# CESNET/GPUJPEG

Measured on AMD Instinct MI355X. Metric: Mpix/s encode+decode (8K RGB q75), higher is better.
Workload: dtype f32

## Files before the change

### gpujpeg_amd/csrc/gj_dec_entropy_tok.hip

```cpp
#include "gj_dec_internal.h"
#include "gj_bitreader.h"

#ifndef GJ_TOK_SUB
#define GJ_TOK_SUB 16
#define GJ_TOK_SUB_MAX 20
#endif
#define GJ_TOK_MAX_SUBS (GJ_TOK_CAP_U / GJ_TOK_SUB + (GJ_TOK_SUB <= 17 ? GJ_TOK_GMAX / 2 : GJ_TOK_GMAX))
#define GJ_TOK_WSTAGE 944
#define GJ_TOK_WG_PER_CU 4
#ifndef GJ_TOK_SYNC
#define GJ_TOK_SYNC 48
#endif
#define GJ_TOK_CHUNK_MAX 48

#ifdef GJ_TRACE_PHASES
static __device__ unsigned long long* gj_trace_buf;
extern "C" GJ_HIP_API int gj_hip_trace_set(void* p) { return hipMemcpyToSymbol(HIP_SYMBOL(gj_trace_buf), &p, sizeof p) == hipSuccess ? 0 : -1; }
#define GJ_TRACE(slot) do { if (threadIdx.x == 0 && gj_trace_buf) gj_trace_buf[(size_t)blockIdx.x * 16 + (slot)] = __builtin_amdgcn_s_memrealtime(); } while (0)
#else
#define GJ_TRACE(slot) ((void)0)
#endif

#ifdef GJ_TOK_STATS
extern "C" GJ_HIP_API unsigned long long gj_tok_stats[64];
unsigned long long gj_tok_stats[64];
#define GJ_STAT_WAVE(sm, i, lane, sym) do { gj_wave_sync(); (sm).statsym[threadIdx.x] = (sym); gj_wave_sync(); if ((lane) == 0) { \
    unsigned long long s_ = 0, m_ = 0; for (int q_ = 0; q_ < 64; q_++) { const unsigned v_ = (sm).statsym[(threadIdx.x & ~63) + q_]; s_ += v_; if (v_ > m_) m_ = v_; } \
    GJ_STAT(i, s_); GJ_STAT((i) + 1, 64 * m_); GJ_STAT((i) + 2, 1); } } while (0)
#define GJ_SYMS(c) (((c) >> 16) + 2u * ((c) & 0xFFFFu))
#define GJ_STAT(i, n) __atomic_fetch_add(&gj_tok_stats[i], (unsigned long long)(n), __ATOMIC_RELAXED)
#else
#define GJ_STAT(i, n) ((void)0)
#define GJ_STAT_WAVE(sm, i, lane, sym) ((void)0)
#endif

#ifndef GJ_TOK_WIN
#define GJ_TOK_WIN 1
#endif
#if GJ_TOK_WIN == 1
#define GJ_TOK_WIN_INIT(sm, p1) uint32_t wcur_ = (p1) >> 5, w0_ = (sm).U[wcur_], w1_ = (sm).U[wcur_ + 1], wnx_ = 0
#define GJ_TOK_WIN_BITS(sm, p1) wnx_ = (sm).U[wcur_ + 2]; const uint32_t win = __builtin_amdgcn_alignbit(w0_, w1_, ~(p1))
#define GJ_TOK_WIN_STEP(p1) do { const uint32_t wn_ = (p1) >> 5; const bool cross_ = wn_ != wcur_; w0_ = cross_ ? w1_ : w0_; w1_ = cross_ ? wnx_ : w1_; wcur_ = wn_; } while (0)
#else
#define GJ_TOK_WIN_INIT(sm, p1) ((void)0)
#define GJ_TOK_WIN_BITS(sm, p1) const uint32_t wi = (p1) >> 5; const uint32_t win = __builtin_amdgcn_alignbit((sm).U[wi], (sm).U[wi + 1], ~(p1))
#define GJ_TOK_WIN_STEP(p1) ((void)0)
#endif


struct GjTokLds {
    uint32_t U[GJ_TOK_CAP_U / 4 + 8];
    __attribute__((aligned(16))) uint16_t tab[2 * GJ_DEC2_WORDS];
    __attribute__((aligned(8))) uint2 rec[GJ_TOK_MAX_SUBS];
    __attribute__((aligned(16))) uint16_t pool[(GJ_TOK_MAX_BLOCKS + GJ_TOK_GMAX) * 2 + 4 * GJ_TOK_WSTAGE];
    uint32_t bb[GJ_TOK_GMAX + 1], cap[GJ_TOK_GMAX + 1], first[GJ_TOK_GMAX];
    uint16_t tabsel[GJ_TOK_GMAX];
    uint32_t sbit[GJ_TOK_GMAX], ebit[GJ_TOK_GMAX], sub0[GJ_TOK_GMAX + 1];
    uint32_t tmp[4];
    uint32_t nwork[2], big;
    uint32_t gpos;
    uint8_t zz[64 + 64];
#ifdef GJ_TOK_STATS
    uint32_t statsym[256];
#endif
};

__device__ __forceinline__ uint32_t gj_tok_run_in(const GjTokLds& sm, const uint32_t from, const uint32_t start_bit)
{
    uint32_t p1 = from - 1u;
    const uint32_t e1 = start_bit - 1u;
    uint32_t z = 1;
    uint32_t toff = (uint32_t)GJ_DEC2_WORDS * 2u;
    GJ_TOK_WIN_INIT(sm, p1);
    while (p1 < e1) {
        GJ_TOK_WIN_BITS(sm, p1);
        const uint16_t* t = reinterpret_cast<const uint16_t*>(reinterpret_cast<const uint8_t*>(sm.tab) + toff);
        uint32_t e = t[gj_bfe_u32<32 - GJ_DEC_FAST_BITS, GJ_DEC_FAST_BITS>(win)];
        if ((e & 31u) == 0) e = t[(e >> 5) + ((win >> 16) & 63u)];
        p1 += e & 31u;
        GJ_TOK_WIN_STEP(p1);
        z += (e >> 9) & 63u;
        const uint32_t inside = (uint32_t)((int32_t)(z - 64u) >> 31);
        z &= inside;
        toff = ((uint32_t)GJ_DEC2_WORDS * 2u) & inside;
    }
    return (p1 - e1) | (z << 5);
}

template <int MODE>
__device__ __forceinline__ uint32_t gj_tok_decode(const GjTokLds& sm, const uint32_t start_bit, const uint32_t end_bit, const uint32_t entry, uint32_t& counts,
                                                  uint16_t* __restrict__ tok_out ,
                                                  uint32_t* __restrict__ s_blkinfo ,
                                                  const uint32_t tok_rel , uint32_t blk,
                                                  const uint32_t nblocks, int16_t* __restrict__ coefs ,
                                                  uint32_t* __restrict__ s_big)
{
    uint32_t p1 = start_bit + (entry & 31u) - 1u;
    const uint32_t e1 = end_bit - 1u;
    uint32_t z = (entry >> 5) & 63u;
    uint32_t toff = z == 0 ? 0u : (uint32_t)GJ_DEC2_WORDS * 2u;
    uint32_t nb = 0, ntok = 0, mx = 0;
    uint16_t* tp = tok_out;
    GJ_TOK_WIN_INIT(sm, p1);
    while (p1 < e1) {
        GJ_TOK_WIN_BITS(sm, p1);
        const uint16_t* t = reinterpret_cast<const uint16_t*>(reinterpret_cast<const uint8_t*>(sm.tab) + toff);
        uint32_t e = t[gj_bfe_u32<32 - GJ_DEC_FAST_BITS, GJ_DEC_FAST_BITS>(win)];
        if ((e & 31u) == 0) e = t[(e >> 5) + ((win >> 16) & 63u)];
        const uint32_t tot = e & 31u, adv = (e >> 9) & 63u, sz = (e >> 5) & 15u;
        if (MODE == 0) {
            ntok += e >> 15;
        } else {
            const uint32_t x = win << (tot - sz);
            uint32_t neg = (uint32_t)((int32_t)~x >> 31);
            GJ_KEEP(neg);
            const uint32_t mag = (x ^ neg) >> ((32u - sz) & 31u);
            const int v = (int)((mag ^ neg) - neg);
            if ((int16_t)e < 0) {
                const uint32_t pos = z + adv - 1u;
                if (MODE == 1) {
                    mx = max(mx, sz);
                    *tp++ = (uint16_t)(((uint32_t)v << 6) | sm.zz[pos]);
                } else {
                    if (blk + nb < nblocks && pos < 64u) coefs[(uint64_t)(blk + nb) * 64 + sm.zz[pos]] = (int16_t)v;
                    ntok++;
                }
            } else if (z == 0) {
                const uint32_t t = MODE == 1 ? tok_rel + (uint32_t)(tp - tok_out) : tok_rel + ntok;
                if (blk + nb <= nblocks) s_blkinfo[blk + nb] = (sz ? (uint32_t)v & 0xFFFFu : 0u) | (t << 16);
            }
        }
        p1 += tot;
        GJ_TOK_WIN_STEP(p1);
        z += adv;
        const uint32_t inside = (uint32_t)((int32_t)(z - 64u) >> 31);
        z &= inside;
        toff = ((uint32_t)GJ_DEC2_WORDS * 2u) & inside;
        nb += 1u + inside;
    }
    if (MODE == 1) ntok = (uint32_t)(tp - tok_out);
    if (MODE == 1 && mx >= 10u) *s_big = 1u;
    counts = nb | (ntok << 16);
    return (p1 - e1) | (z << 5);
}

template <bool COOP>
__global__ __launch_bounds__(256, GJ_TOK_WG_PER_CU) void k_huffman_decode_tok(const gj_geom g, const uint8_t* __restrict__ jpeg, uint64_t jpeg_size,
                                                               const uint32_t* __restrict__ seg_pos, const uint32_t* __restrict__ seg_len,
                                                               const uint32_t* __restrict__ seg_index, const int seg_count_max,
                                                               const uint32_t* __restrict__ seg_count_ptr, const GjBatchPlan plan,
                                                               const uint16_t* __restrict__ tabs, int16_t* __restrict__ coefs,
                                                               uint16_t* __restrict__ d_tok, const uint32_t tok_cap, uint2* __restrict__ d_rec,
                                                               uint32_t* __restrict__ overflow, const GjFold F)
{
    constexpr int CAP_U = GJ_TOK_CAP_U, MAX_BLOCKS = GJ_TOK_MAX_BLOCKS, GMAX = GJ_TOK_GMAX, MAX_SUBS = GJ_TOK_MAX_SUBS;
    if (g.fb.sizes != nullptr) {
        const size_t z = blockIdx.z;
        jpeg += z * g.fb.jpeg;
        jpeg_size = g.fb.sizes[z];
        seg_pos += z * g.fb.seg; seg_len += z * g.fb.seg; seg_index += z * g.fb.seg;
        if (seg_count_ptr) seg_count_ptr += z * (sizeof(gj_scan_summary) / 4);
        overflow += z * (sizeof(gj_scan_summary) / 4);
        coefs += z * g.fb.coefs; d_tok += z * g.fb.tok; d_rec += z * g.fb.rec;
    }
    __shared__ GjTokLds sm;
    constexpr int POOL = sizeof(sm.pool) / 2;
    uint32_t* const s_stage = sm.U + 1;
    uint16_t* const s_pool = sm.pool;
    uint32_t* const s_blkinfo = reinterpret_cast<uint32_t*>(sm.pool);
    uint2* const s_rec = sm.rec;
    uint32_t *const s_bb = sm.bb, *const s_cap = sm.cap, *const s_first = sm.first, *const s_sbit = sm.sbit, *const s_ebit = sm.ebit, *const s_sub0 = sm.sub0;
    uint32_t* const s_tmp = sm.tmp;
    constexpr int BORROW = ((4 * GMAX + 1) * 2 + 7) & ~7;
    uint32_t* const s_pos = reinterpret_cast<uint32_t*>(s_pool + POOL - BORROW);
    uint32_t* const s_len = s_pos + GMAX;
    uint32_t* const s_ubyte = s_len + GMAX;
    uint32_t* const s_ulen = s_ubyte + GMAX + 1;
    static_assert(BORROW <= GJ_TOK_WSTAGE && MAX_SUBS <= POOL - BORROW, "borrowed space");
    uint16_t* const s_work = s_pool;

    const int tid = threadIdx.x, lane = tid & 63, wave = tid >> 6;
    GJ_TRACE(0);
    uint32_t sel_of_lane = 0x0C0C0C0Cu;
    {
        int at = 3;
#pragma unroll
        for (int k = 0; k < 4; k++)
            if (lane & (1 << k)) { sel_of_lane = (sel_of_lane & ~(0xFFu << (8 * at))) | ((uint32_t)k << (8 * at)); at--; }
    }
    if (tid < 128) sm.zz[tid] = tid < 64 ? GJ_ZZ[tid] : 0;
    if (tid == 0) sm.U[0] = 0;
    const uint32_t* end = reinterpret_cast<const uint32_t*>((reinterpret_cast<uintptr_t>(jpeg) + jpeg_size + 3) & ~(uintptr_t)3);

    int pc = 0;
    while (pc + 1 < plan.n && (int)blockIdx.x >= plan.batch0[pc + 1]) pc++;
    const int G = plan.g[pc];
    const int si0 = plan.first[pc] + ((int)blockIdx.x - plan.batch0[pc]) * G;
    uint32_t ld_s = 0xFFFFFFFFu, ld_p = 0, ld_l = 0;
    if (F.recs == nullptr && tid < G && si0 + tid < seg_count_max) { ld_s = seg_index[si0 + tid]; ld_p = seg_pos[si0 + tid]; ld_l = seg_len[si0 + tid]; }
    const int seg_count = seg_count_ptr ? min((int)*seg_count_ptr, seg_count_max) : seg_count_max;
    if (si0 >= seg_count) return;
    const int nseg = min(min(G, plan.first[pc] + plan.count[pc] - si0), seg_count - si0);
    if (F.recs != nullptr) {
        static_assert(GJ_FOLD_SCRATCH_WORDS(GJ_TOK_GMAX) * 2 <= (GJ_TOK_MAX_BLOCKS + GJ_TOK_GMAX) * 2, "fold scratch inside the block slots");
        if (!gj_fold_batch<GJ_TOK_GMAX>(F, g, jpeg, jpeg_size, plan, pc, si0, nseg, reinterpret_cast<uint32_t*>(sm.pool), s_tmp, ld_s, ld_p, ld_l)) return;
    }
    uint32_t loaded_tabs = 0xFFFFFFFFu;
    auto load_tables = [&](const uint32_t tb) {
        const uint4* src0 = reinterpret_cast<const uint4*>(tabs + (tb & 0xFFu) * GJ_DEC2_WORDS);
        const uint4* src1 = reinterpret_cast<const uint4*>(tabs + (tb >> 8) * GJ_DEC2_WORDS);
        uint4* dst = reinterpret_cast<uint4*>(sm.tab);
        for (int t = tid; t < GJ_DEC2_WORDS / 8; t += 256) { dst[t] = src0[t]; dst[GJ_DEC2_WORDS / 8 + t] = src1[t]; }
        loaded_tabs = tb;
    };
    if (plan.n > 1 && plan.n == g.comp_count) load_tables((uint32_t)(g.comp[pc].dc_table * 2 + 0) | ((uint32_t)(g.comp[pc].ac_table * 2 + 1) << 8));
    uint32_t my_pos = 0, my_len = 0, my_nblk = 0;
    {
        uint32_t first = 0, tb = 0;
        if (tid < nseg) {
            const uint32_t s = ld_s, p_ = ld_p, l_ = ld_l;
            if (s < (uint32_t)g.segment_count) {
                const GjSeg sg = gj_segment(g, (int)s);
                const gj_comp_geom& kc = g.comp[sg.comp];
                my_nblk = (uint32_t)sg.nblocks;
                my_pos = p_;
                my_len = l_;
                first = (uint32_t)(kc.data_offset / 64) + (uint32_t)sg.mcu_first;
                tb = (uint32_t)(kc.dc_table * 2 + 0) | ((uint32_t)(kc.ac_table * 2 + 1) << 8);
                if (((my_len + 3u) & ~3u) + 8u > (uint32_t)CAP_U || my_nblk > (uint32_t)MAX_BLOCKS) {
                    *overflow = 1u;
                    my_len = 0;
                    my_nblk = 0;
                }
            }
        }
        if (tid < GMAX) {
            s_first[tid] = first;
            sm.tabsel[tid] = (uint16_t)tb;
        }
        if (wave == 0) {
            s_bb[tid + 1] = gj_wave_incl_scan(tid < nseg ? my_nblk + 1u : 0u);
            s_cap[tid + 1] = gj_wave_incl_scan(my_len ? ((my_len + 3u) & ~3u) + 8u : 0u);
        }
        if (tid == 0) { s_bb[0] = 0; s_cap[0] = 0; sm.nwork[0] = 0; sm.nwork[1] = 0; }
    }
    static_assert(GMAX == 64, "one wave holds the batch's segment table");
    __syncthreads();
    const uint32_t stage0 = (2u * s_bb[nseg] + 7u) & ~7u, stage_cap = (((uint32_t)POOL - stage0) >> 2) & ~7u;
    uint16_t* const stage = s_pool + stage0 + (uint32_t)wave * stage_cap;

    for (int j0 = 0; j0 < nseg;) {
        if (tid == 0) sm.big = 0;
        if (tid < nseg) { s_pos[tid] = my_pos; s_len[tid] = my_len; }
        {
            const unsigned long long mb = __ballot(lane >= j0 && lane < nseg && my_nblk != 0u);
            if (wave == 0 && lane == (mb ? (int)__builtin_ctzll(mb) : j0)) sm.gpos = my_pos;
        }
        const uint32_t tb = sm.tabsel[j0];
        const bool other = lane > j0 && lane < nseg && s_bb[lane + 1] - s_bb[lane] != 1u && sm.tabsel[lane] != tb;
        const unsigned long long mo = __ballot(other);
        const int jstop = mo ? (int)__builtin_ctzll(mo) : nseg;
        const unsigned long long mf = __ballot(lane + 1 > j0 && lane + 1 <= jstop && s_cap[lane + 1] - s_cap[j0] <= (uint32_t)CAP_U);
        const int j1 = max(j0 + 1, mf ? 64 - (int)__builtin_clzll(mf) : 0);
        const int ng = j1 - j0;
        if (COOP) {
            const uint32_t n16 = min((s_cap[j1] - s_cap[j0] + 16u + 4u + 15u) >> 4, (uint32_t)(sizeof(sm.U) / 16));
            uint4* const z = reinterpret_cast<uint4*>(sm.U);
            for (uint32_t t = (uint32_t)tid; t < n16; t += 256u) z[t] = uint4{0u, 0u, 0u, 0u};
        }
        __syncthreads();
        GJ_TRACE(1);

        if (tb != loaded_tabs) load_tables(tb);

        bool coop = false;
        if (COOP) {
            bool irregular = false;
            if (lane < ng) {
                const int j = j0 + lane;
                irregular = s_len[j] == 0 || (lane + 1 < ng && s_pos[j + 1] != s_pos[j] + s_len[j] + 2u);
            }
            const uint32_t A = s_pos[j0], total = s_pos[j1 - 1] + s_len[j1 - 1] - A;
            coop = __ballot(irregular) == 0ull && total <= 256u * GJ_TOK_CHUNK_MAX && A >= 8u && (uint64_t)A + total <= jpeg_size;
        }
        if (coop) {
            const uint32_t A = s_pos[j0], total = s_pos[j1 - 1] + s_len[j1 - 1] - A;
            const uint32_t C = (((total + 255u) >> 8) + 3u) & ~3u;
            const uint32_t off0 = (uint32_t)tid * C;
            const uintptr_t a = reinterpret_cast<uintptr_t>(jpeg) + A + off0;
            const uint32_t* src = reinterpret_cast<const uint32_t*>(a & ~(uintptr_t)3) - 1;
            const uint32_t lead = (uint32_t)((reinterpret_cast<uintptr_t>(jpeg) + A) & 3);
            uint32_t win[GJ_TOK_CHUNK_MAX / 4 + 3];
#pragma unroll
            for (int i = 0; i < GJ_TOK_CHUNK_MAX / 4 + 3; i++) {
                win[i] = 0;
                if ((uint32_t)i < C / 4 + 3u && off0 < total + 4u && src + i < end) win[i] = src[i];
            }
            constexpr int ND = GJ_TOK_CHUNK_MAX / 4;
            uint64_t keep = 0, mark = 0;
            {
                const uint32_t K7 = 0x7F7F7F7Fu, K8 = 0x80808080u;
                uint32_t eq_prev = 0, m2_prev = 0, st_prev = 0;
                uint32_t ffc = 0;
                if (off0 != 0) {
                    const uint32_t x = __builtin_amdgcn_alignbyte(win[1], win[0], lead);
                    ffc = ((x & K7) + 0x01010101u) & x & K8;
                }
#pragma unroll
                for (int i = 0; i <= ND; i++) {
                    if ((uint32_t)(4 * i) <= C) {
                        const uint32_t x = __builtin_amdgcn_alignbyte(win[i + 2], win[i + 1], lead);
                        const uint32_t t = x & K7;
                        const uint32_t eq = (t + 0x01010101u) & x & K8;
                        const uint32_t zr = ~((t + K7) | x) & K8;
                        const uint32_t y = (x ^ 0xD0D0D0D0u) & 0xF8F8F8F8u;
                        const uint32_t rz = ~(((y & K7) + K7) | y) & K8;
                        const uint32_t before = __builtin_amdgcn_alignbit(eq, ffc, 24);
                        ffc = eq;
                        const uint32_t m2 = before & rz, st = before & zr;
                        if (i > 0) {
                            const uint32_t m1 = eq_prev & __builtin_amdgcn_alignbit(m2, m2_prev, 8);
                            const uint32_t kp = K8 & ~(st_prev | m2_prev | m1);
                            keep |= (uint64_t)((((kp >> 7) * 0x01020408u) >> 24) & 15u) << (4 * (i - 1));
                            mark |= (uint64_t)((((m1 >> 7) * 0x01020408u) >> 24) & 15u) << (4 * (i - 1));
                        }
                        eq_prev = eq; m2_prev = m2; st_prev = st;
                    }
                }
                const uint32_t nvalid = off0 >= total ? 0u : min(total - off0, C);
                const uint64_t valid = nvalid >= 64u ? ~0ull : (1ull << nvalid) - 1ull;
                keep &= valid;
                mark &= valid;
            }
            const uint32_t nkeep = (uint32_t)__popcll(keep), nmark = (uint32_t)__popcll(mark);
            uint32_t tot;
            const uint32_t inc = gj_wg256_incl_scan(nkeep | (nmark << 16), s_tmp, &tot);
            uint32_t o = (inc & 0xFFFFu) - nkeep, m = (inc >> 16) - nmark;
            coop = (tot >> 16) == (uint32_t)(ng - 1);
            if (coop) {
#pragma unroll
                for (int i = 0; i < ND; i++) {
                    if ((uint32_t)(4 * i) < C) {
                        const uint32_t x = __builtin_amdgcn_alignbyte(win[i + 2], win[i + 1], lead);
                        const uint32_t nk = (uint32_t)(keep >> (4 * i)) & 15u, nm = (uint32_t)(mark >> (4 * i)) & 15u;
                        const uint32_t below = nm ? ((nm & (0u - nm)) - 1u) : 15u;
                        const uint32_t nA = nk & below, nB = nk & ~below;
                        const uint32_t cA = (uint32_t)__popc(nA);
                        const uint32_t compA = __builtin_amdgcn_perm(0u, x, (uint32_t)__builtin_amdgcn_ds_bpermute((int)(nA << 2), (int)sel_of_lane));
                        const uint32_t compB = __builtin_amdgcn_perm(0u, x, (uint32_t)__builtin_amdgcn_ds_bpermute((int)(nB << 2), (int)sel_of_lane));
                        const uint32_t pA = o + 8u * m, pB = pA + cA + 8u;
                        const uint32_t shA = 8u * (pA & 3u), shB = 8u * (pB & 3u);
                        uint32_t* const dA = s_stage + (pA >> 2);
                        uint32_t* const dB = s_stage + (pB >> 2);
                        atomicOr(dA, compA >> shA);
                        atomicOr(dA + 1, __builtin_amdgcn_alignbit(compA, 0u, shA));
                        atomicOr(dB, compB >> shB);
                        atomicOr(dB + 1, __builtin_amdgcn_alignbit(compB, 0u, shB));
                        uint32_t mm = m;
                        for (uint32_t q = nm; q; q &= q - 1u) {
                            mm++;
                            s_ubyte[j0 + (int)mm] = o + (uint32_t)__popc(nk & ((q & (0u - q)) - 1u)) + 8u * mm;
                        }
                        m = mm;
                        o += (uint32_t)__popc(nk);
                    }
                }
                if (tid == 255) s_ubyte[j1] = o + 8u * m + 8u;
                if (tid == 0) s_ubyte[j0] = 0;
            }
        }
        __syncthreads();
        if (tid == 0) GJ_STAT(coop ? 30 : 31, 1);
        if (coop) {
            if (tid >= j0 && tid < j1) s_ulen[tid] = s_ubyte[tid + 1] - s_ubyte[tid] - 8u;
        } else {
            for (int j = j0 + wave; j < j1; j += 4) {
                const uint32_t len = s_len[j], base = s_cap[j] - s_cap[j0];
                uint32_t ulen = 0;
                if (len) {
                    const uintptr_t a = reinterpret_cast<uintptr_t>(jpeg) + s_pos[j];
                    const uint32_t* src = reinterpret_cast<const uint32_t*>(a & ~(uintptr_t)3);
                    const uint32_t ndw = ((uint32_t)(a & 3) + len + 3u) >> 2;
                    uint32_t w0 = 0;
                    if ((uint32_t)lane < ndw && src + lane < end) w0 = src[lane];
                    ulen = gj_unstuff_segment(jpeg, end, s_pos[j], len, s_stage, base, lane, w0);
                }
                if (lane == 0) { s_ubyte[j] = base; s_ulen[j] = ulen; }
            }
        }
        __syncthreads();

        GJ_TRACE(2);
        uint32_t sub_bytes = GJ_TOK_SUB;
        {
            uint32_t ulen = 0;
            if (tid >= j0 && tid < j1) {
                ulen = my_nblk ? s_ulen[tid] : 0u;
                s_sbit[tid] = s_ubyte[tid] * 8u + 32u;
                s_ebit[tid] = (s_ubyte[tid] + ulen) * 8u + 32u;
            }
            uint32_t tot;
            uint32_t a = gj_wg256_incl_scan(((ulen + GJ_TOK_SUB - 1) / GJ_TOK_SUB) | (ulen << 16), s_tmp, &tot) & 0xFFFFu;
            const uint32_t passes = ((tot & 0xFFFFu) + 255u) >> 8, bytes = tot >> 16;
            if (passes >= 2) {
#pragma unroll
                for (uint32_t s = GJ_TOK_SUB + 1; s <= GJ_TOK_SUB_MAX; s++)
                    if (sub_bytes == GJ_TOK_SUB && bytes / s + (uint32_t)ng <= 256u * (passes - 1u)) sub_bytes = s;
            }
            sub_bytes = (uint32_t)__builtin_amdgcn_readfirstlane((int)sub_bytes);
            if (sub_bytes != GJ_TOK_SUB) a = gj_wg256_incl_scan((ulen + sub_bytes - 1u) / sub_bytes, s_tmp, &tot);
            if (tid >= j0 && tid < j1) s_sub0[tid + 1] = min(a, (uint32_t)MAX_SUBS);
            if (tid == 0) s_sub0[j0] = 0;
        }
        __syncthreads();
        const int nsub = (int)s_sub0[j1];
        const uint32_t sub_bits = sub_bytes * 8u;
        if (tid == 0) { GJ_STAT(32 + min(nsub / 32, 31), 1); GJ_STAT(28, sub_bytes != GJ_TOK_SUB ? 1 : 0); }
        for (int k = tid; k < nsub; k += 256) {
            int lo = j0, hi = j1;
            while (hi - lo > 1) {
                const int mid = (lo + hi) >> 1;
                if (s_sub0[mid] <= (uint32_t)k) lo = mid; else hi = mid;
            }
            s_rec[k].x = (uint32_t)lo << 22;
        }
        __syncthreads();

        GJ_TRACE(3);
        for (int k0 = 0; k0 < nsub; k0 += 256) {
            const int k = k0 + tid;
            uint32_t c0 = 0;
            if (k < nsub) {
                const int j = (int)(s_rec[k].x >> 22);
                const uint32_t i = (uint32_t)k - s_sub0[j];
                const uint32_t sb = s_sbit[j] + i * sub_bits, eb = min(sb + sub_bits, s_ebit[j]);
                const uint32_t e0 = i == 0 ? 0u : gj_tok_run_in(sm, sb - (uint32_t)GJ_TOK_SYNC, sb);
                const uint32_t x0 = gj_tok_decode<0>(sm, sb, eb, e0, c0, nullptr, nullptr, 0, 0, 0, nullptr, nullptr);
                s_rec[k] = make_uint2(e0 | (x0 << 11) | ((uint32_t)j << 22), c0);
            }
            GJ_STAT_WAVE(sm, 16, lane, GJ_SYMS(c0));
        }
        GJ_TRACE(4);
        for (int round = 0;; round++) {
            __syncthreads();
            uint32_t* const cnt = &sm.nwork[round & 1];
            for (int k0 = 0; k0 < nsub; k0 += 256) {
                const int k = k0 + tid;
                bool cand = false;
                if (k < nsub) {
                    const uint32_t x = s_rec[k].x;
                    cand = (uint32_t)k != s_sub0[x >> 22] && ((s_rec[k - 1].x >> 11) & 0x7FFu) != (x & 0x7FFu);
                }
                const unsigned long long m = __ballot(cand);
                uint32_t base = 0;
                if (lane == 0 && m) base = atomicAdd(cnt, (uint32_t)__popcll(m));
                base = (uint32_t)__builtin_amdgcn_readfirstlane((int)base);
                if (cand) s_work[base + (uint32_t)__popcll(m & ((1ull << lane) - 1ull))] = (uint16_t)k;
            }
            __syncthreads();
            const int nwork = (int)*cnt;
            if (tid == 0) { GJ_STAT(0, round == 0 ? nsub : 0); GJ_STAT(1 + min(round, 13), nwork); GJ_STAT(15, nwork == 0 ? round : 0); }
            if (tid == 0) sm.nwork[(round + 1) & 1] = 0;
            if (nwork == 0) break;
            for (int w = tid; w < nwork; w += 256) {
                const int k = s_work[w];
                const int j = (int)(s_rec[k].x >> 22);
                const uint32_t i = (uint32_t)k - s_sub0[j];
                const uint32_t sb = s_sbit[j] + i * sub_bits, eb = min(sb + sub_bits, s_ebit[j]);
                const uint32_t e = (s_rec[k - 1].x >> 11) & 0x7FFu;
                uint32_t c;
                const uint32_t x = gj_tok_decode<0>(sm, sb, eb, e, c, nullptr, nullptr, 0, 0, 0, nullptr, nullptr);
                s_rec[k] = make_uint2(e | (x << 11) | ((uint32_t)j << 22), c);
            }
        }

        GJ_TRACE(5);
        {
            uint32_t carry = 0;
            for (int k0 = 0; k0 < nsub; k0 += 256) {
                const int k = k0 + tid;
                const uint32_t v = k < nsub ? s_rec[k].y : 0;
                uint32_t tot;
                const uint32_t inc = gj_wg256_incl_scan(v, s_tmp, &tot);
                __syncthreads();
                if (k < nsub) s_rec[k].y = carry + inc;
                carry += tot;
            }
        }
        for (uint32_t b = s_bb[j0] + (uint32_t)tid; b < s_bb[j1]; b += 256) s_blkinfo[b] = 0xFFFF0000u;
        __syncthreads();

        GJ_TRACE(6);
        const uint32_t T = nsub > 0 ? s_rec[nsub - 1].y >> 16 : 0u;
        uint32_t gbase = 4u * sm.gpos;
        if (sm.gpos > tok_cap / 4u || T > tok_cap - gbase) gbase = 0xFFFFFFFFu;
        if (gbase != 0xFFFFFFFFu) {
            const int ka = (int)(((uint32_t)nsub * (uint32_t)wave) >> 2), kb = (int)(((uint32_t)nsub * (uint32_t)(wave + 1)) >> 2);
            for (int k0 = ka; k0 < kb;) {
                const uint32_t P0 = k0 > 0 ? s_rec[k0 - 1].y >> 16 : 0u;
                const uint32_t a0 = (gbase + P0) & 7u;
                const int kk = k0 + lane;
                const bool fits = kk < kb && a0 + ((s_rec[min(kk, nsub - 1)].y >> 16) - P0) <= stage_cap;
                const unsigned long long fm = __ballot(fits);
                const int n = fm == ~0ull ? 64 : __builtin_ctzll(~fm);
                gj_wave_sync();
                uint32_t c = 0;
                if (lane < n) {
                    const int j = (int)(s_rec[kk].x >> 22);
                    const uint32_t kf = s_sub0[j];
                    const uint32_t i = (uint32_t)kk - kf;
                    const uint32_t before_k = kk > 0 ? s_rec[kk - 1].y : 0u, before_f = kf > 0 ? s_rec[kf - 1].y : 0u;
                    const uint32_t sb = s_sbit[j] + i * sub_bits, eb = min(sb + sub_bits, s_ebit[j]);
                    gj_tok_decode<1>(sm, sb, eb, s_rec[kk].x & 0x7FFu, c, stage + a0 + ((before_k >> 16) - P0), s_blkinfo + s_bb[j], before_k >> 16,
                                     (before_k & 0xFFFFu) - (before_f & 0xFFFFu), s_bb[j + 1] - s_bb[j] - 1u, nullptr, &sm.big);
                }
                gj_wave_sync();
                GJ_STAT_WAVE(sm, 20, lane, GJ_SYMS(c));
                const uint32_t cnt = (s_rec[k0 + n - 1].y >> 16) - P0;
                uint16_t* const dst = d_tok + (size_t)(gbase + P0 - a0);
                for (uint32_t p = (uint32_t)lane; p * 8u < a0 + cnt; p += 64) {
                    const uint32_t lo = p * 8u, hi = lo + 8u;
                    if (lo >= a0 && hi <= a0 + cnt) {
                        *reinterpret_cast<uint4*>(dst + lo) = *reinterpret_cast<const uint4*>(stage + lo);
                    } else {
                        for (uint32_t s = max(lo, a0); s < min(hi, a0 + cnt); s++) dst[s] = stage[s];
                    }
                }
                k0 += n;
                if (lane == 0) { GJ_STAT(24, 1); GJ_STAT(25, n); GJ_STAT(26, k0 >= kb ? (kb - ka + 63) / 64 : 0); GJ_STAT(27, k0 >= kb ? 1 : 0); }
            }
        }
        __syncthreads();

        GJ_TRACE(7);
        const bool planes = sm.big != 0 || gbase == 0xFFFFFFFFu;
        if (planes) {
            for (int j = j0 + wave; j < j1; j += 4) {
                const uint32_t chunks = (s_bb[j + 1] - s_bb[j] - 1u) * 8u;
                for (uint32_t c = (uint32_t)lane; c < chunks; c += 64)
                    reinterpret_cast<uint4*>(coefs + (uint64_t)(s_first[j] + (c >> 3)) * 64)[c & 7u] = make_uint4(0, 0, 0, 0);
            }
            __syncthreads();
            for (int k = tid; k < nsub; k += 256) {
                const int j = (int)(s_rec[k].x >> 22);
                const uint32_t kf = s_sub0[j];
                const uint32_t i = (uint32_t)k - kf;
                const uint32_t before_k = k > 0 ? s_rec[k - 1].y : 0u, before_f = kf > 0 ? s_rec[kf - 1].y : 0u;
                const uint32_t sb = s_sbit[j] + i * sub_bits, eb = min(sb + sub_bits, s_ebit[j]);
                uint32_t c;
                gj_tok_decode<2>(sm, sb, eb, s_rec[k].x & 0x7FFu, c, nullptr, s_blkinfo + s_bb[j], 0, (before_k & 0xFFFFu) - (before_f & 0xFFFFu),
                                 s_bb[j + 1] - s_bb[j] - 1u, coefs + (uint64_t)s_first[j] * 64, nullptr);
            }
            __syncthreads();
        }

        for (int j = j0 + wave; j < j1; j += 4) {
            const uint32_t bb = s_bb[j];
            const int nblk = (int)(s_bb[j + 1] - bb) - 1;
            const uint32_t k_end = s_sub0[j + 1];
            const uint32_t seg_end = k_end > s_sub0[j] ? s_rec[k_end - 1].y >> 16 : 0u;
            int carry = 0;
            for (int kb0 = 0; kb0 < nblk; kb0 += 64) {
                const int kb = kb0 + lane;
                const uint32_t info = kb < nblk ? s_blkinfo[bb + kb] : 0xFFFF0000u;
                const uint32_t inc = gj_wave_incl_scan((uint32_t)(int)(int16_t)(info & 0xFFFFu));
                const int dc = carry + (int)inc;
                carry += (int)(uint32_t)__builtin_amdgcn_readlane((int)inc, 63);
                if (kb < nblk) {
                    const uint32_t r = s_first[j] + (uint32_t)kb;
                    if (planes) {
                        coefs[(uint64_t)r * 64] = (int16_t)dc;
                        d_rec[r] = make_uint2(0u, 0xFFFF0000u);
                    } else {
                        const uint32_t t0 = info >> 16, nx = s_blkinfo[bb + kb + 1] >> 16;
                        const uint32_t t1 = nx != 0xFFFFu ? nx : seg_end;
                        const bool seen = t0 != 0xFFFFu;
                        const uint32_t cnt = seen && t1 >= t0 ? min(t1 - t0, 63u) : 0u;
                        d_rec[r] = make_uint2(seen ? gbase + t0 : 0u, (cnt << 16) | ((uint32_t)dc & 0xFFFFu));
                    }
                }
            }
        }
        __syncthreads();
        GJ_TRACE(8);
        j0 = j1;
    }
}

void gj_launch_huffman_tok(const gj_dec_job* job, hipStream_t st)
{
    const gj_geom& g = job->g;
    const unsigned frames = job->batch.count > 1 ? job->batch.count : 1u;
    const GjBatchPlan plan = gj_plan_batches(job, GJ_TOK_CAP_U, GJ_TOK_MAX_BLOCKS, GJ_TOK_GMAX, frames > 1 ? 0u : GJ_TOK_RESIDENT);
    auto kernel = job->tune.dec_tok_nocoop ? k_huffman_decode_tok<false> : k_huffman_decode_tok<true>;
    GjFold F = {nullptr, nullptr, 0, 0, 0, nullptr, nullptr};
    const bool fold = gj_tok_folds_table(job);
    if (fold) {
        const gj_scan_deferred& sc = job->scan;
        F = GjFold{sc.recs, sc.lists, sc.wgs, sc.part_bytes, sc.begin, sc.h_summary, sc.h_maxlen_parts};
        *sc.maxlen_part_count = (uint32_t)plan.batch0[plan.n];
    }
    hipLaunchKernelGGL(kernel, dim3((unsigned)plan.batch0[plan.n], 1, frames), dim3(256), 0, st, g, job->d_jpeg, job->jpeg_size, job->d_seg_pos, job->d_seg_len, job->d_seg_index,
                       job->seg_count, fold ? nullptr : job->d_seg_count, plan, job->d_huff_tab2, job->d_coefs, (uint16_t*)job->d_tok, job->tok_cap, (uint2*)job->d_blkrec,
                       job->d_overflow, F);
}

bool gj_tok_folds_table(const gj_dec_job* job)
{
    const gj_geom& g = job->g;
    if (!job->scan.valid || job->batch.count > 1 || g.fb.sizes != nullptr || g.interleaved || g.restart_interval <= 0 || job->seg_count != g.segment_count) return false;
    if (job->scan.wgs > 256u || job->scan.h_summary == nullptr || job->scan.h_maxlen_parts == nullptr || job->scan.maxlen_part_count == nullptr) return false;
    const GjBatchPlan plan = gj_plan_batches(job, GJ_TOK_CAP_U, GJ_TOK_MAX_BLOCKS, GJ_TOK_GMAX, GJ_TOK_RESIDENT);
    return plan.n == g.comp_count && (uint32_t)plan.batch0[plan.n] <= job->scan.maxlen_capacity;
}
```

Measured before the change: 171,400.

## Interleave two sub-stream Huffman counting passes per thread in token decoder

When a group holds more than 256 sub-streams, the first counting pass now gives each thread two sub-streams and decodes them in lockstep within one loop. This replaces several serial 256-wide rounds, cutting the trip count and giving the LDS table lookups two independent chains to overlap. In exchange it adds register pressure, extra work for a frozen reader once its stream ends, and divergence when the two streams differ in length. Step-count tracing and extra stats hooks are also added, but they compile out by default.

```diff
diff --git a/gpujpeg_amd/csrc/gj_dec_entropy_tok.hip b/gpujpeg_amd/csrc/gj_dec_entropy_tok.hip
--- a/gpujpeg_amd/csrc/gj_dec_entropy_tok.hip
+++ b/gpujpeg_amd/csrc/gj_dec_entropy_tok.hip
@@ -12,26 +12,52 @@
 #define GJ_TOK_SYNC 48
 #endif
 #define GJ_TOK_CHUNK_MAX 48
+#ifndef GJ_TOK_PAIR
+#define GJ_TOK_PAIR 1
+#endif
+#ifndef GJ_TOK_PAIR_MIN
+#define GJ_TOK_PAIR_MIN 256
+#endif
 
 #ifdef GJ_TRACE_PHASES
 static __device__ unsigned long long* gj_trace_buf;
 extern "C" GJ_HIP_API int gj_hip_trace_set(void* p) { return hipMemcpyToSymbol(HIP_SYMBOL(gj_trace_buf), &p, sizeof p) == hipSuccess ? 0 : -1; }
 #define GJ_TRACE(slot) do { if (threadIdx.x == 0 && gj_trace_buf) gj_trace_buf[(size_t)blockIdx.x * 16 + (slot)] = __builtin_amdgcn_s_memrealtime(); } while (0)
+#define GJ_TRACE_STEPS(slot, n) do { const uint32_t m_ = gj_wave_max(n); if (threadIdx.x == 0 && gj_trace_buf) gj_trace_buf[(size_t)blockIdx.x * 16 + (slot)] += m_; } while (0)
+__device__ __forceinline__ uint32_t gj_wave_max(const uint32_t v)
+{
+    uint32_t m = 0;
+    bool in = true;
+    for (int b = 15; b >= 0; b--) {
+        const bool has = in && ((v >> b) & 1u);
+        if (__ballot(has)) { m |= 1u << b; in = has; }
+    }
+    return m;
+}
 #else
 #define GJ_TRACE(slot) ((void)0)
-#endif
-
+#define GJ_TRACE_STEPS(slot, n) ((void)(n))
+#endif
+
+#define GJ_SYMS(c) (((c) >> 16) + 2u * ((c) & 0xFFFFu))
 #ifdef GJ_TOK_STATS
 extern "C" GJ_HIP_API unsigned long long gj_tok_stats[64];
 unsigned long long gj_tok_stats[64];
 #define GJ_STAT_WAVE(sm, i, lane, sym) do { gj_wave_sync(); (sm).statsym[threadIdx.x] = (sym); gj_wave_sync(); if ((lane) == 0) { \
     unsigned long long s_ = 0, m_ = 0; for (int q_ = 0; q_ < 64; q_++) { const unsigned v_ = (sm).statsym[(threadIdx.x & ~63) + q_]; s_ += v_; if (v_ > m_) m_ = v_; } \
     GJ_STAT(i, s_); GJ_STAT((i) + 1, 64 * m_); GJ_STAT((i) + 2, 1); } } while (0)
-#define GJ_SYMS(c) (((c) >> 16) + 2u * ((c) & 0xFFFFu))
 #define GJ_STAT(i, n) __atomic_fetch_add(&gj_tok_stats[i], (unsigned long long)(n), __ATOMIC_RELAXED)
+extern "C" GJ_HIP_API unsigned int gj_tok_nsub_hist[GJ_TOK_MAX_SUBS + 1], gj_tok_pair_passes, gj_tok_plane_groups;
+unsigned int gj_tok_nsub_hist[GJ_TOK_MAX_SUBS + 1], gj_tok_pair_passes, gj_tok_plane_groups;
+#define GJ_STAT_NSUB(n) __atomic_fetch_add(&gj_tok_nsub_hist[n], 1u, __ATOMIC_RELAXED)
+#define GJ_STAT_PAIR() __atomic_fetch_add(&gj_tok_pair_passes, 1u, __ATOMIC_RELAXED)
+#define GJ_STAT_PLANES() __atomic_fetch_add(&gj_tok_plane_groups, 1u, __ATOMIC_RELAXED)
 #else
 #define GJ_STAT(i, n) ((void)0)
-#define GJ_STAT_WAVE(sm, i, lane, sym) ((void)0)
+#define GJ_STAT_NSUB(n) ((void)0)
+#define GJ_STAT_PAIR() ((void)0)
+#define GJ_STAT_PLANES() ((void)0)
+#define GJ_STAT_WAVE(sm, i, lane, sym) ((void)(sym))
 #endif
 
 #ifndef GJ_TOK_WIN
@@ -65,7 +91,7 @@
 #endif
 };
 
-__device__ __forceinline__ uint32_t gj_tok_run_in(const GjTokLds& sm, const uint32_t from, const uint32_t start_bit)
+__device__ __forceinline__ uint32_t gj_tok_run_in(const GjTokLds& sm, const uint32_t from, const uint32_t start_bit, uint32_t& steps )
 {
     uint32_t p1 = from - 1u;
     const uint32_t e1 = start_bit - 1u;
@@ -83,6 +109,7 @@
         const uint32_t inside = (uint32_t)((int32_t)(z - 64u) >> 31);
         z &= inside;
         toff = ((uint32_t)GJ_DEC2_WORDS * 2u) & inside;
+        steps++;
     }
     return (p1 - e1) | (z << 5);
 }
@@ -93,7 +120,7 @@
                                                   uint32_t* __restrict__ s_blkinfo ,
                                                   const uint32_t tok_rel , uint32_t blk,
                                                   const uint32_t nblocks, int16_t* __restrict__ coefs ,
-                                                  uint32_t* __restrict__ s_big)
+                                                  uint32_t* __restrict__ s_big, uint32_t& steps )
 {
     uint32_t p1 = start_bit + (entry & 31u) - 1u;
     const uint32_t e1 = end_bit - 1u;
@@ -137,12 +164,93 @@
         z &= inside;
         toff = ((uint32_t)GJ_DEC2_WORDS * 2u) & inside;
         nb += 1u + inside;
+        steps++;
     }
     if (MODE == 1) ntok = (uint32_t)(tp - tok_out);
     if (MODE == 1 && mx >= 10u) *s_big = 1u;
     counts = nb | (ntok << 16);
     return (p1 - e1) | (z << 5);
 }
+
+#if GJ_TOK_PAIR && GJ_TOK_WIN == 1
+struct GjTokStream {
+    uint32_t from, start, end;
+    uint32_t entry, exit, counts;
+};
+struct GjTokReader { uint32_t p1, z, toff, cnt, w0, w1, wnx, wcur; };
+
+__device__ __forceinline__ void gj_tok_reader_step(GjTokReader& r, const uint32_t e)
+{
+    r.p1 += e & 31u;
+    const uint32_t wn = r.p1 >> 5;
+    const bool cross = wn != r.wcur;
+    r.w0 = cross ? r.w1 : r.w0;
+    r.w1 = cross ? r.wnx : r.w1;
+    r.wcur = wn;
+    r.z += (e >> 9) & 63u;
+    const uint32_t inside = (uint32_t)((int32_t)(r.z - 64u) >> 31);
+    r.z &= inside;
+    r.toff = ((uint32_t)GJ_DEC2_WORDS * 2u) & inside;
+    r.cnt += ((e & 0x8000u) << 1) + 1u + inside;
+}
+
+__device__ __forceinline__ void gj_tok_pair_loop(const GjTokLds& sm, GjTokReader& A, GjTokReader& B, const uint32_t endA1, const uint32_t endB1, uint32_t& steps)
+{
+    static_assert((32 + 8 * GJ_TOK_CAP_U + 30) / 32 + 2 < (int)(sizeof(GjTokLds::U) / 4), "a frozen reader's look-ahead stays in the stage");
+    const uint8_t* const tab = reinterpret_cast<const uint8_t*>(sm.tab);
+    while (A.p1 < endA1 || B.p1 < endB1) {
+        const uint32_t actA = (uint32_t)((int32_t)(A.p1 - endA1) >> 31), actB = (uint32_t)((int32_t)(B.p1 - endB1) >> 31);
+        A.wnx = sm.U[A.wcur + 2];
+        B.wnx = sm.U[B.wcur + 2];
+        const uint32_t winA = __builtin_amdgcn_alignbit(A.w0, A.w1, ~A.p1), winB = __builtin_amdgcn_alignbit(B.w0, B.w1, ~B.p1);
+        const uint16_t* const tA = reinterpret_cast<const uint16_t*>(tab + A.toff);
+        const uint16_t* const tB = reinterpret_cast<const uint16_t*>(tab + B.toff);
+        uint32_t eA = tA[gj_bfe_u32<32 - GJ_DEC_FAST_BITS, GJ_DEC_FAST_BITS>(winA)];
+        uint32_t eB = tB[gj_bfe_u32<32 - GJ_DEC_FAST_BITS, GJ_DEC_FAST_BITS>(winB)];
+        if ((((eA & 31u) == 0) | ((eB & 31u) == 0)) != 0) {
+            if ((eA & 31u) == 0) eA = tA[(eA >> 5) + ((winA >> 16) & 63u)];
+            if ((eB & 31u) == 0) eB = tB[(eB >> 5) + ((winB >> 16) & 63u)];
+        }
+        gj_tok_reader_step(A, eA & actA);
+        gj_tok_reader_step(B, eB & actB);
+        steps++;
+    }
+}
+
+__device__ __forceinline__ void gj_tok_reader_init(const GjTokLds& sm, GjTokReader& r, const GjTokStream& s)
+{
+    r.p1 = s.from - 1u;
+    r.z = s.from != s.start ? 1u : 0u;
+    r.toff = r.z ? (uint32_t)GJ_DEC2_WORDS * 2u : 0u;
+    r.cnt = 0;
+    r.wcur = r.p1 >> 5;
+    r.w0 = sm.U[r.wcur];
+    r.w1 = sm.U[r.wcur + 1];
+    r.wnx = 0;
+}
+
+__device__ __forceinline__ void gj_tok_count2(const GjTokLds& sm, GjTokStream& A, GjTokStream& B, uint32_t& steps)
+{
+    GjTokReader a, b;
+    gj_tok_reader_init(sm, a, A);
+    gj_tok_reader_init(sm, b, B);
+    gj_tok_pair_loop(sm, a, b, A.start - 1u, B.start - 1u, steps);
+    A.entry = (a.p1 - (A.start - 1u)) | (a.z << 5);
+    B.entry = (b.p1 - (B.start - 1u)) | (b.z << 5);
+    a.toff = a.z == 0 ? 0u : (uint32_t)GJ_DEC2_WORDS * 2u;
+    b.toff = b.z == 0 ? 0u : (uint32_t)GJ_DEC2_WORDS * 2u;
+    a.cnt = 0;
+    b.cnt = 0;
+    gj_tok_pair_loop(sm, a, b, A.end - 1u, B.end - 1u, steps);
+    A.exit = (a.p1 - (A.end - 1u)) | (a.z << 5);
+    B.exit = (b.p1 - (B.end - 1u)) | (b.z << 5);
+    A.counts = a.cnt;
+    B.counts = b.cnt;
+}
+#define GJ_TOK_PAIRED 1
+#else
+#define GJ_TOK_PAIRED 0
+#endif
 
 template <bool COOP>
 __global__ __launch_bounds__(256, GJ_TOK_WG_PER_CU) void k_huffman_decode_tok(const gj_geom g, const uint8_t* __restrict__ jpeg, uint64_t jpeg_size,
@@ -415,7 +523,7 @@
         __syncthreads();
         const int nsub = (int)s_sub0[j1];
         const uint32_t sub_bits = sub_bytes * 8u;
-        if (tid == 0) { GJ_STAT(32 + min(nsub / 32, 31), 1); GJ_STAT(28, sub_bytes != GJ_TOK_SUB ? 1 : 0); }
+        if (tid == 0) { GJ_STAT(32 + min(nsub / 32, 31), 1); GJ_STAT(28, sub_bytes != GJ_TOK_SUB ? 1 : 0); GJ_STAT_NSUB(nsub); }
         for (int k = tid; k < nsub; k += 256) {
             int lo = j0, hi = j1;
             while (hi - lo > 1) {
@@ -427,19 +535,60 @@
         __syncthreads();
 
         GJ_TRACE(3);
-        for (int k0 = 0; k0 < nsub; k0 += 256) {
-            const int k = k0 + tid;
-            uint32_t c0 = 0;
-            if (k < nsub) {
-                const int j = (int)(s_rec[k].x >> 22);
-                const uint32_t i = (uint32_t)k - s_sub0[j];
-                const uint32_t sb = s_sbit[j] + i * sub_bits, eb = min(sb + sub_bits, s_ebit[j]);
-                const uint32_t e0 = i == 0 ? 0u : gj_tok_run_in(sm, sb - (uint32_t)GJ_TOK_SYNC, sb);
-                const uint32_t x0 = gj_tok_decode<0>(sm, sb, eb, e0, c0, nullptr, nullptr, 0, 0, 0, nullptr, nullptr);
-                s_rec[k] = make_uint2(e0 | (x0 << 11) | ((uint32_t)j << 22), c0);
-            }
-            GJ_STAT_WAVE(sm, 16, lane, GJ_SYMS(c0));
-        }
+        uint32_t steps1 = 0;
+        for (int b0 = 0; b0 < nsub;) {
+            const int rem = nsub - b0;
+            const int P = rem > 256 ? 256 : (GJ_TOK_PAIRED && rem > GJ_TOK_PAIR_MIN ? (rem + 1) >> 1 : rem);
+            const int n = GJ_TOK_PAIRED ? min(rem, 2 * P) : P;
+            uint32_t syms = 0;
+#if GJ_TOK_PAIRED
+            if (n > P) {
+                if (tid == 0) GJ_STAT_PAIR();
+                if (tid < P) {
+                    const int kA = b0 + tid, kB = kA + P;
+                    const bool hasB = kB < b0 + n;
+                    const int jA = (int)(s_rec[kA].x >> 22);
+                    const uint32_t iA = (uint32_t)kA - s_sub0[jA];
+                    GjTokStream A, B;
+                    A.start = s_sbit[jA] + iA * sub_bits;
+                    A.end = min(A.start + sub_bits, s_ebit[jA]);
+                    A.from = iA == 0 ? A.start : A.start - (uint32_t)GJ_TOK_SYNC;
+                    int jB = 0;
+                    B.from = B.start = B.end = 32u;
+                    if (hasB) {
+                        jB = (int)(s_rec[kB].x >> 22);
+                        const uint32_t iB = (uint32_t)kB - s_sub0[jB];
+                        B.start = s_sbit[jB] + iB * sub_bits;
+                        B.end = min(B.start + sub_bits, s_ebit[jB]);
+                        B.from = iB == 0 ? B.start : B.start - (uint32_t)GJ_TOK_SYNC;
+                    }
+                    gj_tok_count2(sm, A, B, steps1);
+                    s_rec[kA] = make_uint2(A.entry | (A.exit << 11) | ((uint32_t)jA << 22), A.counts);
+                    if (hasB) s_rec[kB] = make_uint2(B.entry | (B.exit << 11) | ((uint32_t)jB << 22), B.counts);
+                    syms = GJ_SYMS(A.counts) + GJ_SYMS(B.counts);
+                    GJ_STAT(19, (iA != 0 && A.end - A.start <= 32u ? 1 : 0) + (hasB && B.from != B.start && B.end - B.start <= 32u ? 1 : 0));
+                    GJ_STAT(23, (iA == 0 && A.end - A.start < (uint32_t)GJ_TOK_SYNC ? 1 : 0) + (hasB && B.from == B.start && B.end - B.start < (uint32_t)GJ_TOK_SYNC ? 1 : 0));
+                    GJ_STAT(29, hasB && GJ_SYMS(B.counts) != 0 && GJ_SYMS(A.counts) != 0 && (GJ_SYMS(A.counts) > 3u * GJ_SYMS(B.counts) || GJ_SYMS(B.counts) > 3u * GJ_SYMS(A.counts)) ? 1 : 0);
+                }
+            } else
+#endif
+            {
+                const int k = b0 + tid;
+                if (tid < n) {
+                    uint32_t c0 = 0;
+                    const int j = (int)(s_rec[k].x >> 22);
+                    const uint32_t i = (uint32_t)k - s_sub0[j];
+                    const uint32_t sb = s_sbit[j] + i * sub_bits, eb = min(sb + sub_bits, s_ebit[j]);
+                    const uint32_t e0 = i == 0 ? 0u : gj_tok_run_in(sm, sb - (uint32_t)GJ_TOK_SYNC, sb, steps1);
+                    const uint32_t x0 = gj_tok_decode<0>(sm, sb, eb, e0, c0, nullptr, nullptr, 0, 0, 0, nullptr, nullptr, steps1);
+                    s_rec[k] = make_uint2(e0 | (x0 << 11) | ((uint32_t)j << 22), c0);
+                    syms = GJ_SYMS(c0);
+                }
+            }
+            GJ_STAT_WAVE(sm, 16, lane, syms);
+            b0 += n;
+        }
+        if (wave == 0) { GJ_TRACE_STEPS(9, steps1); GJ_TRACE_STEPS(11, tid == 0 ? (uint32_t)nsub : 0u); }
         GJ_TRACE(4);
         for (int round = 0;; round++) {
             __syncthreads();
@@ -468,8 +617,8 @@
                 const uint32_t i = (uint32_t)k - s_sub0[j];
                 const uint32_t sb = s_sbit[j] + i * sub_bits, eb = min(sb + sub_bits, s_ebit[j]);
                 const uint32_t e = (s_rec[k - 1].x >> 11) & 0x7FFu;
-                uint32_t c;
-                const uint32_t x = gj_tok_decode<0>(sm, sb, eb, e, c, nullptr, nullptr, 0, 0, 0, nullptr, nullptr);
+                uint32_t c, steps = 0;
+                const uint32_t x = gj_tok_decode<0>(sm, sb, eb, e, c, nullptr, nullptr, 0, 0, 0, nullptr, nullptr, steps);
                 s_rec[k] = make_uint2(e | (x << 11) | ((uint32_t)j << 22), c);
             }
         }
@@ -494,6 +643,7 @@
         const uint32_t T = nsub > 0 ? s_rec[nsub - 1].y >> 16 : 0u;
         uint32_t gbase = 4u * sm.gpos;
         if (sm.gpos > tok_cap / 4u || T > tok_cap - gbase) gbase = 0xFFFFFFFFu;
+        uint32_t steps5 = 0;
         if (gbase != 0xFFFFFFFFu) {
             const int ka = (int)(((uint32_t)nsub * (uint32_t)wave) >> 2), kb = (int)(((uint32_t)nsub * (uint32_t)(wave + 1)) >> 2);
             for (int k0 = ka; k0 < kb;) {
@@ -512,7 +662,7 @@
                     const uint32_t before_k = kk > 0 ? s_rec[kk - 1].y : 0u, before_f = kf > 0 ? s_rec[kf - 1].y : 0u;
                     const uint32_t sb = s_sbit[j] + i * sub_bits, eb = min(sb + sub_bits, s_ebit[j]);
                     gj_tok_decode<1>(sm, sb, eb, s_rec[kk].x & 0x7FFu, c, stage + a0 + ((before_k >> 16) - P0), s_blkinfo + s_bb[j], before_k >> 16,
-                                     (before_k & 0xFFFFu) - (before_f & 0xFFFFu), s_bb[j + 1] - s_bb[j] - 1u, nullptr, &sm.big);
+                                     (before_k & 0xFFFFu) - (before_f & 0xFFFFu), s_bb[j + 1] - s_bb[j] - 1u, nullptr, &sm.big, steps5);
                 }
                 gj_wave_sync();
                 GJ_STAT_WAVE(sm, 20, lane, GJ_SYMS(c));
@@ -530,11 +680,13 @@
                 if (lane == 0) { GJ_STAT(24, 1); GJ_STAT(25, n); GJ_STAT(26, k0 >= kb ? (kb - ka + 63) / 64 : 0); GJ_STAT(27, k0 >= kb ? 1 : 0); }
             }
         }
+        if (wave == 0) GJ_TRACE_STEPS(10, steps5);
         __syncthreads();
 
         GJ_TRACE(7);
         const bool planes = sm.big != 0 || gbase == 0xFFFFFFFFu;
         if (planes) {
+            if (tid == 0) GJ_STAT_PLANES();
             for (int j = j0 + wave; j < j1; j += 4) {
                 const uint32_t chunks = (s_bb[j + 1] - s_bb[j] - 1u) * 8u;
                 for (uint32_t c = (uint32_t)lane; c < chunks; c += 64)
@@ -547,9 +699,9 @@
                 const uint32_t i = (uint32_t)k - kf;
                 const uint32_t before_k = k > 0 ? s_rec[k - 1].y : 0u, before_f = kf > 0 ? s_rec[kf - 1].y : 0u;
                 const uint32_t sb = s_sbit[j] + i * sub_bits, eb = min(sb + sub_bits, s_ebit[j]);
-                uint32_t c;
+                uint32_t c, steps = 0;
                 gj_tok_decode<2>(sm, sb, eb, s_rec[k].x & 0x7FFu, c, nullptr, s_blkinfo + s_bb[j], 0, (before_k & 0xFFFFu) - (before_f & 0xFFFFu),
-                                 s_bb[j + 1] - s_bb[j] - 1u, coefs + (uint64_t)s_first[j] * 64, nullptr);
+                                 s_bb[j + 1] - s_bb[j] - 1u, coefs + (uint64_t)s_first[j] * 64, nullptr, steps);
             }
             __syncthreads();
         }
```

New measurement: 170,100. About the same (-0.8%).
